# mfkiwl/GPS-JAMMING

Hardware: AMD Instinct MI355X
Metric: Msamples/s uint8 I/Q through PSD+TDOA xcorr (higher is better)
Workload: dtype f32

## Files before the change

gps-jamming_amd/csrc/k_scan.hip:

```cpp
#include <type_traits>

#include "gj_common.h"

namespace gj {

constexpr int kScanThreads = 256;
constexpr size_t kScanTile = 65536;

__device__ __forceinline__ void acc_moments(const uint4& q, unsigned& s2, unsigned& s1) {
    s2 = __builtin_amdgcn_udot4(q.x, q.x, s2, false);
    s2 = __builtin_amdgcn_udot4(q.y, q.y, s2, false);
    s2 = __builtin_amdgcn_udot4(q.z, q.z, s2, false);
    s2 = __builtin_amdgcn_udot4(q.w, q.w, s2, false);
    s1 = __builtin_amdgcn_udot4(q.x, 0x01010101u, s1, false);
    s1 = __builtin_amdgcn_udot4(q.y, 0x01010101u, s1, false);
    s1 = __builtin_amdgcn_udot4(q.z, 0x01010101u, s1, false);
    s1 = __builtin_amdgcn_udot4(q.w, 0x01010101u, s1, false);
}

__device__ __forceinline__ void block_byte_moments(const uint8_t* __restrict__ p, size_t begin, size_t end,
                                                   unsigned long long& s2_out, unsigned long long& s1_out) {
    __shared__ unsigned long long red[2][kScanThreads / 64];
    const int tid = threadIdx.x;
    unsigned s2 = 0, s1 = 0;
    size_t a0 = (begin + 15) & ~size_t(15);
    size_t a1 = end & ~size_t(15);
    if (a0 > a1) { a0 = end; a1 = end; }
    if (begin + tid < a0) { unsigned u = p[begin + tid]; s2 += u * u; s1 += u; }
    if (a1 + tid < end && a1 >= a0) { unsigned u = p[a1 + tid]; s2 += u * u; s1 += u; }
    const uint4* v = reinterpret_cast<const uint4*>(p + a0);
    const size_t nvec = (a1 - a0) >> 4;
    size_t i = tid;
    for (; i + 3 * kScanThreads < nvec; i += 4 * kScanThreads) {
        uint4 w0 = v[i], w1 = v[i + kScanThreads], w2 = v[i + 2 * kScanThreads], w3 = v[i + 3 * kScanThreads];
        acc_moments(w0, s2, s1); acc_moments(w1, s2, s1); acc_moments(w2, s2, s1); acc_moments(w3, s2, s1);
    }
    for (; i < nvec; i += kScanThreads) {
        uint4 w0 = v[i];
        acc_moments(w0, s2, s1);
    }
    unsigned long long t2 = wave_sum_u64(s2), t1 = wave_sum_u64(s1);
    if ((tid & 63) == 0) { red[0][tid >> 6] = t2; red[1][tid >> 6] = t1; }
    __syncthreads();
    if (tid == 0) {
        s2_out = red[0][0] + red[0][1] + red[0][2] + red[0][3];
        s1_out = red[1][0] + red[1][1] + red[1][2] + red[1][3];
    }
    __syncthreads();
}

__device__ __forceinline__ float power_from_moments(unsigned long long s2, unsigned long long s1, size_t npairs,
                                                    float eps, int o2) {
    const long long S = 4ll * (long long)s2 - 4ll * o2 * (long long)s1 + (long long)o2 * o2 * (long long)(2 * npairs);
    const float mean = (float)((double)S / (4.0 * (double)npairs));
    return mean + eps;
}

__device__ __forceinline__ float power_from_msum(unsigned long long S, size_t npairs, float eps) {
    const float mean = (float)((double)S / (4.0 * (double)npairs));
    return mean + eps;
}

__global__ __launch_bounds__(kScanThreads) void chunk_power_kernel(const uint8_t* __restrict__ iq, size_t nbytes,
                                                                   size_t chunk_bytes, unsigned tiles_per_chunk,
                                                                   float eps, int flags, float* __restrict__ power,
                                                                   unsigned long long* __restrict__ acc, int o2) {
    const size_t c = blockIdx.x / tiles_per_chunk;
    const unsigned t = blockIdx.x % tiles_per_chunk;
    const size_t off = c * chunk_bytes;
    const size_t len = (nbytes - off < chunk_bytes) ? nbytes - off : chunk_bytes;
    const size_t npairs = len >> 1;
    if ((flags & GJ_CP_ODD_CHUNK_ZERO) && ((len & 1) || len == 0)) {
        if (t == 0 && threadIdx.x == 0) power[c] = 0.0f;
        return;
    }
    if (npairs == 0) {
        if (t == 0 && threadIdx.x == 0) power[c] = __builtin_nanf("");
        return;
    }
    const size_t use_end = off + 2 * npairs;
    size_t b = off + (size_t)t * kScanTile;
    size_t e = b + kScanTile;
    if (e > use_end) e = use_end;
    if (b > e) b = e;
    unsigned long long s2 = 0, s1 = 0;
    block_byte_moments(iq, b, e, s2, s1);
    if (threadIdx.x == 0) {
        if (tiles_per_chunk == 1) {
            power[c] = power_from_moments(s2, s1, npairs, eps, o2);
        } else {
            atomicAdd(&acc[2 * c], s2);
            atomicAdd(&acc[2 * c + 1], s1);
        }
    }
}

__global__ void chunk_power_finalize_kernel(const unsigned long long* __restrict__ acc, size_t nchunks, size_t nbytes,
                                            size_t chunk_bytes, float eps, int flags, float* __restrict__ power,
                                            int o2, bool msum = false) {
    const size_t c = blockIdx.x * (size_t)blockDim.x + threadIdx.x;
    if (c >= nchunks) return;
    const size_t off = c * chunk_bytes;
    const size_t len = (nbytes - off < chunk_bytes) ? nbytes - off : chunk_bytes;
    const size_t npairs = len >> 1;
    if ((flags & GJ_CP_ODD_CHUNK_ZERO) && ((len & 1) || len == 0)) return;
    if (npairs == 0) return;
    power[c] = msum ? power_from_msum(acc[2 * c], npairs, eps) : power_from_moments(acc[2 * c], acc[2 * c + 1], npairs, eps, o2);
}

int launch_chunk_power(gj_ctx* ctx, const uint8_t* d_iq, size_t nbytes, size_t chunk_bytes, float eps, int flags,
                       float* d_power) {
    if (chunk_bytes == 0) return fail(ctx, GJ_ERR_INVALID, "chunk_bytes must be > 0");
    const size_t nchunks = gj_chunk_count(nbytes, chunk_bytes);
    if (nchunks == 0) return GJ_OK;
    const size_t tiles = (chunk_bytes + kScanTile - 1) / kScanTile;
    if (nchunks * tiles > 0x7fffffffull) return fail(ctx, GJ_ERR_UNSUPPORTED, "too many tiles");
    unsigned long long* acc = nullptr;
    if (tiles > 1) {
        int rc = ensure_workspace(ctx, nchunks * 16);
        if (rc) return rc;
        acc = reinterpret_cast<unsigned long long*>(ctx->ws);
        GJ_HIP(ctx, hipMemsetAsync(acc, 0, nchunks * 16, ctx->stream));
    }
    hipLaunchKernelGGL(chunk_power_kernel, dim3((unsigned)(nchunks * tiles)), dim3(kScanThreads), 0, ctx->stream, d_iq,
                       nbytes, chunk_bytes, (unsigned)tiles, eps, flags, d_power, acc, ctx->off2);
    GJ_LAUNCH_CHECK(ctx);
    if (tiles > 1) {
        hipLaunchKernelGGL(chunk_power_finalize_kernel, dim3((unsigned)((nchunks + 255) / 256)), dim3(256), 0,
                           ctx->stream, acc, nchunks, nbytes, chunk_bytes, eps, flags, d_power, ctx->off2);
        GJ_LAUNCH_CHECK(ctx);
    }
    return GJ_OK;
}

__device__ __forceinline__ unsigned float_key(float f) {
    unsigned b = __float_as_uint(f);
    return (b & 0x80000000u) ? ~b : (b | 0x80000000u);
}
__device__ __forceinline__ float key_float(unsigned k) {
    return __uint_as_float((k & 0x80000000u) ? (k & 0x7fffffffu) : ~k);
}

constexpr int kThrThreads = 256;
constexpr int kThrPerThread = 64;
constexpr int kThrCache = kThrThreads * kThrPerThread;

struct ThrShared {
    unsigned hist[256];
    unsigned wave_tot[4];
    unsigned digit, rest;
    unsigned nan_flag;
    unsigned count_le;
    unsigned next_key;
    unsigned long long above;
// ... 183 lines not shown

constexpr size_t kAmpTileSamples = kScanTile / 2;

struct AmpTile {
    double sum;
    long long first;
};

__device__ double block_sum_f64(double v, double* sh ) {
    v = wave_sum_f64(v);
    __syncthreads();
    if ((threadIdx.x & 63) == 0) sh[threadIdx.x >> 6] = v;
    __syncthreads();
    double t = 0.0;
    for (unsigned k = 0; k < blockDim.x / 64; ++k) t += sh[k];
    return t;
}

__device__ long long amp_block_first(const AmpTile* __restrict__ tiles, size_t ntiles, long long* first_s) {
    if (threadIdx.x == 0) *first_s = 0x7fffffffffffffffll;
    __syncthreads();
    long long f = 0x7fffffffffffffffll;
    for (size_t t = threadIdx.x; t < ntiles; t += 16 * (size_t)blockDim.x) {
        long long v[16];
#pragma unroll
        for (int k = 0; k < 16; ++k) {
            const size_t tt = t + (size_t)k * blockDim.x;
            v[k] = tt < ntiles ? tiles[tt].first : 0x7fffffffffffffffll;
        }
#pragma unroll
        for (int k = 0; k < 16; ++k) f = v[k] < f ? v[k] : f;
    }
    if (f != 0x7fffffffffffffffll) atomicMin(first_s, f);
    __syncthreads();
    return *first_s;
}

__device__ double amp_block_tail(const uint8_t* __restrict__ iq, size_t nsamples, const AmpTile* __restrict__ tiles,
                                 long long first, Unpack up, double* sh) {
    const size_t t0 = (size_t)first / kAmpTileSamples;
    if ((size_t)first == t0 * kAmpTileSamples) return tiles[t0].sum;
    const size_t e0 = ((t0 + 1) * kAmpTileSamples < nsamples) ? (t0 + 1) * kAmpTileSamples : nsamples;
    double acc = 0.0;
    for (size_t s = (size_t)first + threadIdx.x; s < e0; s += blockDim.x) acc += (double)amp_of(iq[2 * s], iq[2 * s + 1], up);
    return block_sum_f64(acc, sh);
}

__device__ double amp_block_total(const AmpTile* __restrict__ tiles, size_t ntiles, size_t t0, double* sh) {
    double acc = 0.0;
    for (size_t t = t0 + 1 + threadIdx.x; t < ntiles; t += 16 * (size_t)blockDim.x) {
        double v[16];
#pragma unroll
        for (int k = 0; k < 16; ++k) {
            const size_t tt = t + (size_t)k * blockDim.x;
            v[k] = tt < ntiles ? tiles[tt].sum : 0.0;
        }
#pragma unroll
        for (int g = 0; g < 2; ++g) {
            if (t + (size_t)(8 * g) * blockDim.x < ntiles)
                acc += ((v[8 * g] + v[8 * g + 1]) + (v[8 * g + 2] + v[8 * g + 3])) + ((v[8 * g + 4] + v[8 * g + 5]) + (v[8 * g + 6] + v[8 * g + 7]));
        }
    }
    return block_sum_f64(acc, sh);
}

static inline bool power_edge_value(size_t nchunks, size_t nbytes, size_t chunk_bytes, int flags, float* val) {
    if (!nchunks) return false;
    const size_t len = nbytes - (nchunks - 1) * chunk_bytes;
    if ((flags & GJ_CP_ODD_CHUNK_ZERO) && (len & 1)) { *val = 0.0f; return true; }
    if ((len >> 1) == 0) { *val = __builtin_nanf(""); return true; }
    return false;
}
__device__ __forceinline__ void amp_combine_body(const AmpTile* __restrict__ tiles, size_t ntiles,
                                                 const gj_amp_part* __restrict__ parts, int n_parts, size_t nsamples,
                                                 gj_amp_stats* __restrict__ out, double* sh) {
    long long first = 0x7fffffffffffffffll;
    double tail = 0.0;
    for (int p = 0; p < n_parts; ++p)
        if (parts[p].first_index >= 0 && parts[p].first_index < first) { first = parts[p].first_index; tail = parts[p].tail; }
    if (first == 0x7fffffffffffffffll) {
        if (threadIdx.x == 0) {
            out->first_index = -1; out->count = 0; out->sum = 0.0; out->mean = 0.f; out->reserved = 0.f;
        }
        return;
    }
    const double behind = amp_block_total(tiles, ntiles, (size_t)first / kAmpTileSamples, sh);
    if (threadIdx.x == 0) {
        const double total = behind + tail;
        const unsigned long long cnt = nsamples - (size_t)first;
        out->first_index = first;
        out->count = cnt;
        out->sum = total;
        out->mean = (float)(total / (double)cnt);
        out->reserved = 0.f;
    }
}

__global__ __launch_bounds__(256) void amp_combine_kernel(const AmpTile* __restrict__ tiles, size_t ntiles,
                                                           const gj_amp_part* __restrict__ parts, int n_parts,
                                                           size_t nsamples, gj_amp_stats* __restrict__ out) {
    __shared__ double sh[16];
    amp_combine_body(tiles, ntiles, parts, n_parts, nsamples, out, sh);
}

__global__ __launch_bounds__(kThrThreads) __attribute__((amdgpu_num_vgpr(104))) void combine_stats_kernel(
    const gj_combine_capture* __restrict__ caps, int n_captures, float pct, float ratio) {
    __shared__ ThrShared sh_thr;
    __shared__ double sh_amp[16];
    const int b = blockIdx.x;
    if (b < n_captures) {
        const gj_combine_capture c = caps[b];
        power_threshold_body(c.d_power, (size_t)c.n_chunks, pct, ratio, c.d_stats, nullptr, sh_thr);
    } else {
        const gj_combine_capture c = caps[b - n_captures];
        amp_combine_body(static_cast<const AmpTile*>(c.d_tiles), (size_t)c.n_tiles, c.d_amp_parts, c.n_parts,
                         (size_t)(c.total_bytes / 2), c.d_amp, sh_amp);
        if (threadIdx.x == 0) onset_combine(c.d_onset_parts, c.n_parts, c.d_onset);
    }
}

int launch_combine_stats(gj_ctx* ctx, const gj_combine_capture* d_caps, int n_captures, float pct, float rise_db) {
    const float ratio = (float)pow(10.0, (double)rise_db / 10.0);
    hipLaunchKernelGGL(combine_stats_kernel, dim3(2u * (unsigned)n_captures), dim3(kThrThreads), 0, ctx->stream, d_caps,
                       n_captures, pct, ratio);
    GJ_LAUNCH_CHECK(ctx);
    return GJ_OK;
}

constexpr int kOnsetOut = 2048;
constexpr int kOnsetMaxWin = 8192;

struct OnsetScratch {
    unsigned long long noise_S;
    float noise;
    float thr;
};

constexpr double kOnsetGuard = 1e-6;

__device__ __forceinline__ int onset_pad(int k) { return k + (k >> 5); }

typedef short gj_short2 __attribute__((ext_vector_type(2)));

__device__ __forceinline__ int wave_sum_lane63(int v) {
    v += __builtin_amdgcn_update_dpp(0, v, 0xB1, 0xf, 0xf, false);
    v += __builtin_amdgcn_update_dpp(0, v, 0x4E, 0xf, 0xf, false);
    v += __builtin_amdgcn_update_dpp(0, v, 0x141, 0xf, 0xf, false);
    v += __builtin_amdgcn_update_dpp(0, v, 0x140, 0xf, 0xf, false);
    v += __builtin_amdgcn_update_dpp(0, v, 0x142, 0xa, 0xf, false);
    v += __builtin_amdgcn_update_dpp(0, v, 0x143, 0xc, 0xf, false);
    return v;
}


template <bool TRACK_FIRST>
__global__ __launch_bounds__(kScanThreads) void stream_scan_kernel(const uint8_t* __restrict__ iq, size_t nsamples,
                                                                   size_t nbytes, size_t chunk_bytes,
                                                                   unsigned tiles_per_chunk, float eps, int flags,
                                                                   float* __restrict__ power,
                                                                   unsigned long long* __restrict__ acc, float thr,
                                                                   AmpTile* __restrict__ tiles,
                                                                   unsigned* __restrict__ cblk, Unpack up,
                                                                   unsigned skip_tiles, unsigned tile_base,
                                                                   unsigned noise_block, const uint8_t* __restrict__ noise_src,
                                                                   int noise_samples, OnsetScratch* __restrict__ sc) {
    if (blockIdx.x == noise_block) {
        unsigned long long s2 = 0, s1 = 0;
        block_byte_moments(noise_src, 0, (size_t)2 * noise_samples, s2, s1);
        if (threadIdx.x == 0)
            sc->noise_S = (unsigned long long)(4ll * (long long)s2 - 4ll * up.off2 * (long long)s1 + (long long)up.off2 * up.off2 * (2ll * noise_samples));
        return;
    }
    __shared__ unsigned long long red_m[2][kScanThreads / 64];
    __shared__ double red_s[kScanThreads / 64];
    __shared__ long long red_f[kScanThreads / 64];
    const int tid = threadIdx.x;
    const size_t t = (size_t)blockIdx.x + tile_base;
    const size_t b0 = t * kScanTile;
    const size_t use_end = 2 * nsamples;
    const size_t b1 = (b0 + kScanTile < use_end) ? b0 + kScanTile : use_end;
    const size_t nvec = (b1 - b0) >> 4;
    const uint4* v = reinterpret_cast<const uint4*>(iq + b0);
    unsigned S = 0;
    double sum = 0.0;
    long long first = 0x7fffffffffffffffll;
    unsigned k2 = 0x00020002u, km255 = pk_minus_off2(up.off2);
    asm volatile("" : "+v"(k2), "+v"(km255));
    auto body = [&](const uint4& q, unsigned i, const bool live) {
        const unsigned ws[4] = {q.x, q.y, q.z, q.w};
        int m[8];
#pragma unroll
        for (int k = 0; k < 4; ++k) {
            m[2 * k] = msq_of_half<0>(ws[k], k2, km255);
            m[2 * k + 1] = msq_of_half<1>(ws[k], k2, km255);
        }
        float part = 0.f;
#pragma unroll
        for (int k = 0; k < 8; ++k) {
            const float r = __fsqrt_rn((float)m[k]);
            part += r;
            if constexpr (TRACK_FIRST) {
                const long long idx = (long long)((b0 >> 1) + (size_t)i * 8 + k);
                if (live && r * up.half_scale > thr && idx < first) first = idx;
            }
        }
        const unsigned m8 = live ? (unsigned)(((m[0] + m[1]) + (m[2] + m[3])) + ((m[4] + m[5]) + (m[6] + m[7]))) : 0u;
        S += m8;
        const int c512 = wave_sum_lane63((int)m8);
        if ((tid & 63) == 63) cblk[(b0 >> 10) + (i >> 6)] = (unsigned)c512;
        sum += (double)(live ? part : 0.f);
    };
    if (nvec == kScanTile / 16) {
        for (unsigned i = tid; i < (unsigned)(kScanTile / 16); i += 4 * kScanThreads) {
            const uint4 q0 = v[i], q1 = v[i + kScanThreads], q2 = v[i + 2 * kScanThreads], q3 = v[i + 3 * kScanThreads];
            body(q0, i, true);
            body(q1, i + kScanThreads, true);
            body(q2, i + 2 * kScanThreads, true);
            body(q3, i + 3 * kScanThreads, true);
        }
    } else {
        const unsigned lane = tid & 63;
        for (unsigned ib = (unsigned)tid - lane; ib < (unsigned)nvec; ib += kScanThreads) {
            const unsigned i = ib + lane;
            const bool live = i < (unsigned)nvec;
            const uint4 q = live ? v[i] : uint4{0u, 0u, 0u, 0u};
            body(q, i, live);
        }
    }
    if (tid == 0 && (b0 + (nvec << 4)) < b1) {
        unsigned c = 0;
        for (size_t n = (b0 >> 1) + nvec * 8; 2 * n < b1; ++n) {
            const unsigned ui = iq[2 * n], uq = iq[2 * n + 1];
            const unsigned mm = m_of(ui, uq, up.off2);
            S += mm;
            c += mm;
            const float r = __fsqrt_rn((float)mm);
            sum += (double)r;
            if (TRACK_FIRST && r * up.half_scale > thr && (long long)n < first) first = (long long)n;
        }
        (void)c;
    }
    if (b1 == use_end && (b1 & 1023) != 0) {
        __syncthreads();
        if (tid < 64) {
            const size_t jb = (b1 - 1) >> 10;
            int c = 0;
            for (size_t n = jb * 512 + tid; n < nsamples; n += 64) c += (int)m_of(iq[2 * n], iq[2 * n + 1], up.off2);
            c = group_sum_dpp<64>(c);
            if (tid == 0) cblk[jb] = (unsigned)c;
        }
    }
    if constexpr (!TRACK_FIRST) {
        if (tid == 0 && b1 > b0) first = (long long)(b0 >> 1);
    }
    const unsigned long long mS = wave_sum_u64(S);
    sum = wave_sum_f64(sum);
#pragma unroll
    for (int off = 32; off > 0; off >>= 1) {
        const long long o = __shfl_xor(first, off, 64);
        first = o < first ? o : first;
    }
    if ((tid & 63) == 0) { red_m[0][tid >> 6] = mS; red_s[tid >> 6] = sum; red_f[tid >> 6] = first; }
    __syncthreads();
    if (tid == 0 && t >= skip_tiles) {
        const unsigned long long tS = red_m[0][0] + red_m[0][1] + red_m[0][2] + red_m[0][3];
        AmpTile at;
        at.sum = ((red_s[0] + red_s[1]) + (red_s[2] + red_s[3])) * (double)up.half_scale;
        long long f = red_f[0];
        for (int k = 1; k < 4; ++k) f = red_f[k] < f ? red_f[k] : f;
        at.first = (f == 0x7fffffffffffffffll) ? f : f - (long long)((size_t)skip_tiles * (kScanTile / 2));
        const size_t to = t - skip_tiles;
        tiles[to] = at;
        const size_t c = to / tiles_per_chunk;
        const size_t off = c * chunk_bytes;
        const size_t len = (nbytes - off < chunk_bytes) ? nbytes - off : chunk_bytes;
        const bool zero_rule = (flags & GJ_CP_ODD_CHUNK_ZERO) && ((len & 1) || len == 0);
        if (tiles_per_chunk == 1) {
            power[c] = zero_rule ? 0.0f : ((len >> 1) ? power_from_msum(tS, len >> 1, eps) : __builtin_nanf(""));
        } else {
            atomicAdd(&acc[2 * c], tS);
        }
    }
}

constexpr size_t kTailSlotBytes = 256u << 10;
constexpr size_t kTailPrioBytes = 256u << 20;
constexpr int kTailBlocks = 2048;
constexpr int kTailHalo = (kOnsetMaxWin + 510) / 512 + 1;
constexpr int kTailPre = kTailBlocks + kTailHalo + (kTailBlocks + kTailHalo) / 32 + 8;

struct TailRec {
    unsigned long long first;
    unsigned long long guard;
    unsigned below;
    unsigned pad;
};

struct TailArgs {
    const uint8_t* iq;
    unsigned long long nsamples;
    long long sample0;
    unsigned long long total_samples;
    unsigned long long slot_nsamples;
    int has_thr, is_part, valid, has_slot, hi_prio;
    float* power;
    unsigned long long nchunks;
    float pct, ratio;
    float* stats;
    uint8_t* mask;
    const uint8_t* own_iq;
    unsigned long long own_samples, own_tiles;
    const AmpTile* tiles;
    gj_amp_stats* amp;
    gj_amp_part* amp_part;
    long long own_sample0;
    int window, noise_samples, noise_in_scratch;
    float factor;
    const unsigned* cblk;
    OnsetScratch* sc;
    TailRec* rec;
    unsigned* arrive;
    unsigned nct;
    gj_onset* onset;
    uint8_t* slot;
    unsigned long long slice_samples;
    Unpack up;
};

struct TailShared {
    unsigned long long r64[2][kScanThreads / 64];
    unsigned r32[kScanThreads / 64];
    unsigned long long b64[2];
    unsigned b32;
    int last;
    long long start;
};

__device__ __forceinline__ unsigned long long block_min_u64(unsigned long long v, TailShared& sh, int slot) {
#pragma unroll
    for (int off = 32; off > 0; off >>= 1) {
        const unsigned long long o = __shfl_xor(v, off, 64);
        v = o < v ? o : v;
    }
    if ((threadIdx.x & 63) == 0) sh.r64[slot][threadIdx.x >> 6] = v;
    __syncthreads();
    unsigned long long r = sh.r64[slot][0];
#pragma unroll
    for (int k = 1; k < kScanThreads / 64; ++k) r = sh.r64[slot][k] < r ? sh.r64[slot][k] : r;
    __syncthreads();
    return r;
}
__device__ __forceinline__ unsigned block_max_u32(unsigned v, TailShared& sh) {
#pragma unroll
    for (int off = 32; off > 0; off >>= 1) {
        const unsigned o = __shfl_xor(v, off, 64);
        v = o > v ? o : v;
    }
    if ((threadIdx.x & 63) == 0) sh.r32[threadIdx.x >> 6] = v;
    __syncthreads();
    unsigned r = sh.r32[0];
#pragma unroll
    for (int k = 1; k < kScanThreads / 64; ++k) r = sh.r32[k] > r ? sh.r32[k] : r;
    __syncthreads();
    return r;
}
__device__ __forceinline__ unsigned long long block_sum_u64(unsigned long long v, TailShared& sh) {
    v = wave_sum_u64(v);
    if ((threadIdx.x & 63) == 0) sh.r64[0][threadIdx.x >> 6] = v;
    __syncthreads();
    unsigned long long r = 0;
#pragma unroll
    for (int k = 0; k < kScanThreads / 64; ++k) r += sh.r64[0][k];
    __syncthreads();
    return r;
}

__device__ __forceinline__ void block_min2_max(unsigned long long& a, unsigned long long& b, unsigned& c, TailShared& sh) {
#pragma unroll
    for (int off = 32; off > 0; off >>= 1) {
        const unsigned long long oa = __shfl_xor(a, off, 64), ob = __shfl_xor(b, off, 64);
        const unsigned oc = __shfl_xor(c, off, 64);
        a = oa < a ? oa : a;
        b = ob < b ? ob : b;
        c = oc > c ? oc : c;
    }
    if ((threadIdx.x & 63) == 0) { sh.r64[0][threadIdx.x >> 6] = a; sh.r64[1][threadIdx.x >> 6] = b; sh.r32[threadIdx.x >> 6] = c; }
    __syncthreads();
    a = sh.r64[0][0]; b = sh.r64[1][0]; c = sh.r32[0];
#pragma unroll
    for (int k = 1; k < kScanThreads / 64; ++k) {
        a = sh.r64[0][k] < a ? sh.r64[0][k] : a;
        b = sh.r64[1][k] < b ? sh.r64[1][k] : b;
        c = sh.r32[k] > c ? sh.r32[k] : c;
// ... 118 lines not shown
            }
        }
        unsigned long long hit = best, hit_lo = best_lo;
        unsigned b = 0;
#pragma unroll
        for (int i = 0; i < kOnsetOut / kScanThreads; ++i) {
            const int k = tid + i * kScanThreads;
            if (k < npos && o0 + k < best) b = Sv[i] > b ? Sv[i] : b;
        }
        block_min2_max(hit, hit_lo, b, sh);
        if (hit != ~0ull) {
            b = 0;
#pragma unroll
            for (int i = 0; i < kOnsetOut / kScanThreads; ++i) {
                const int k = tid + i * kScanThreads;
                if (k < npos && o0 + k < hit) b = Sv[i] > b ? Sv[i] : b;
            }
            b = block_max_u32(b, sh);
        }
        below = b > below ? b : below;
        if (hit_lo != ~0ull && guard == ~0ull) guard = hit_lo;
        if (hit != ~0ull) { first = hit; break; }
        kstart = k1 + (npos + 511) / 512;
    }
    if (tid == 0) {
        TailRec r;
        r.first = first; r.guard = guard; r.below = below; r.pad = 0;
        A.rec[w] = r;
    }
}

__device__ void tail_onset_finish(const TailArgs& A, TailShared& sh) {
    const int tid = threadIdx.x;
    const int window = A.window;
    if (A.valid) {
        unsigned long long wmin = ~0ull;
        for (unsigned w = tid; w < A.nct; w += kScanThreads)
            if (A.rec[w].first != ~0ull) { wmin = w; break; }
        const unsigned long long wstar = block_min_u64(wmin, sh, 0);
        const bool found = wstar != ~0ull;
        const unsigned wlast = found ? (unsigned)wstar : A.nct - 1;
        unsigned below = 0;
        unsigned long long guard = ~0ull;
        for (unsigned w = tid; w <= wlast; w += kScanThreads) {
            const TailRec r = A.rec[w];
            below = r.below > below ? r.below : below;
            guard = r.guard < guard ? r.guard : guard;
        }
        below = block_max_u32(below, sh);
        guard = block_min_u64(guard, sh, 1);
        const unsigned long long i0 = found ? A.rec[wstar].first : 0ull;
        unsigned long long S = 0;
        if (found)
            for (int k = tid; k < window; k += kScanThreads) S += m_of(A.iq[2 * (i0 + k)], A.iq[2 * (i0 + k) + 1], A.up.off2);
        S = block_sum_u64(S, sh);
        if (tid == 0) {
            const double thr = (double)A.sc->thr, scale = 0.25 / (double)window;
            gj_onset o;
            o.start_index = found ? A.sample0 + (long long)i0 + window / 2 : -1;
            o.noise_power = A.sc->noise;
            o.threshold = A.sc->thr;
            o.margin_hit = found ? (float)(((double)S * scale - thr) / thr) : 0.f;
            o.margin_before = (float)((thr - (double)below * scale) / thr);
            unsigned long long ig = guard;
            if (found && i0 < ig) ig = i0;
            o.guard_index = ig != ~0ull ? A.sample0 + (long long)ig + window / 2 : -1;
            *A.onset = o;
            sh.start = o.start_index;
        }
    } else if (tid == 0) {
        gj_onset o;
        o.start_index = -1; o.noise_power = 0.f; o.threshold = 0.f; o.margin_hit = 0.f; o.margin_before = 0.f; o.guard_index = -1;
        *A.onset = o;
        sh.start = -1;
    }
    __syncthreads();
    if (A.has_slot)
        tdoa_slot_body(A.iq, (size_t)A.slot_nsamples, sh.start, (size_t)A.slice_samples, A.slot, A.sample0, (size_t)A.total_samples,
                       (size_t)tid, (size_t)kScanThreads, tid == 0);
}

__global__ __launch_bounds__(kScanThreads) void scan_tail_kernel(TailArgs A) {
    __shared__ ThrShared sh_thr;
    __shared__ double sh_amp[16];
    __shared__ long long first_s;
    __shared__ TailShared sh;
    __shared__ unsigned pre_c[kTailPre];
    __shared__ unsigned thread_tot[kScanThreads];
    extern __shared__ unsigned pre_x[];
    const int tid = threadIdx.x;
    unsigned b = blockIdx.x;
    if (A.hi_prio) __builtin_amdgcn_s_setprio(3);
    if (A.has_thr) {
        if (b == 0) {
            power_threshold_body(A.power, (size_t)A.nchunks, A.pct, A.ratio, A.stats, A.mask, sh_thr);
            return;
        }
        --b;
    }
    if (b == 0) {
        const long long first = amp_block_first(A.tiles, (size_t)A.own_tiles, &first_s);
        if (first == 0x7fffffffffffffffll) {
            if (tid == 0) {
                if (A.is_part) { A.amp_part->first_index = -1; A.amp_part->count = 0; A.amp_part->sum = 0.0; A.amp_part->tail = 0.0; }
                else { A.amp->first_index = -1; A.amp->count = 0; A.amp->sum = 0.0; A.amp->mean = 0.f; A.amp->reserved = 0.f; }
            }
            return;
        }
        const double tail = amp_block_tail(A.own_iq, (size_t)A.own_samples, A.tiles, first, A.up, sh_amp);
        const double behind = amp_block_total(A.tiles, (size_t)A.own_tiles, (size_t)first / kAmpTileSamples, sh_amp);
        if (tid == 0) {
            const unsigned long long cnt = A.own_samples - (size_t)first;
            if (A.is_part) {
                A.amp_part->first_index = A.own_sample0 + first;
                A.amp_part->count = cnt;
                A.amp_part->sum = behind + tail;
                A.amp_part->tail = tail;
            } else {
                const double total = behind + tail;
                A.amp->first_index = first;
                A.amp->count = cnt;
                A.amp->sum = total;
                A.amp->mean = (float)(total / (double)cnt);
                A.amp->reserved = 0.f;
            }
        }
        return;
    }
    --b;
    if (A.valid) tail_onset_range(A, b, pre_c, thread_tot, pre_x, sh);
    if (tid == 0) {
        const unsigned ticket = arrive_release(A.arrive);
        const int last = ticket == A.nct - 1;
        if (last) last_arriver_acquire(A.arrive);
        sh.last = last;
    }
    __syncthreads();
    if (!sh.last) return;
    tail_onset_finish(A, sh);
}

struct ScanPart {
    size_t halo_bytes;
    long long buf_sample0;
    const uint8_t* d_noise;
    size_t total_samples;
    AmpTile* d_tiles;
    gj_amp_part* d_amp;
};

struct ScanState {
    const uint8_t* d_iq;
    size_t nbytes, chunk_bytes, own_bytes, nsamples, own_samples, ntiles, skip, own_tiles, nchunks, tpc, noise_bytes;
    float eps, rssi_threshold, factor;
    int flags, noise_samples, window, valid;
    bool noise_here, track, is_part;
    float* d_power;
    gj_amp_stats* d_amp;
    gj_onset* d_onset;
    ScanPart part;
    size_t off_tiles, off_acc, off_blk, off_rec;
    unsigned nct;
};
static_assert(sizeof(ScanState) <= sizeof(ScanJob::state), "ScanJob::state too small");

bool scan_fusable(const uint8_t* d_iq, size_t nbytes, size_t chunk_bytes) {
    return chunk_bytes >= kScanTile && chunk_bytes % kScanTile == 0 && (reinterpret_cast<uintptr_t>(d_iq) & 15) == 0 && nbytes >= 2;
}

static int scan_begin_impl(gj_ctx* ctx, const uint8_t* d_iq, size_t nbytes, size_t chunk_bytes, float eps, int flags,
                           float* d_power, float rssi_threshold, gj_amp_stats* d_amp, int noise_samples, int window,
                           float factor, gj_onset* d_onset, const ScanPart* part, ScanJob& job) {
    if (noise_samples <= 0 || window <= 0) return fail(ctx, GJ_ERR_INVALID, "noise_samples and window must be > 0");
    if (window > kOnsetMaxWin) return fail(ctx, GJ_ERR_UNSUPPORTED, "window > %d", kOnsetMaxWin);
    ScanState st;
    memset(&st, 0, sizeof(st));
    st.d_iq = d_iq; st.nbytes = nbytes; st.chunk_bytes = chunk_bytes; st.eps = eps; st.flags = flags; st.d_power = d_power;
    st.rssi_threshold = rssi_threshold; st.d_amp = d_amp; st.noise_samples = noise_samples; st.window = window;
    st.factor = factor; st.d_onset = d_onset;
    st.is_part = part != nullptr;
    if (part) st.part = *part;
    const size_t halo = part ? part->halo_bytes : 0;
    st.own_bytes = nbytes - halo;
    st.nsamples = nbytes / 2;
    st.own_samples = st.own_bytes / 2;
    st.ntiles = (2 * st.nsamples + kScanTile - 1) / kScanTile;
    st.skip = halo / kScanTile;
    st.own_tiles = st.ntiles - st.skip;
    st.nchunks = gj_chunk_count(st.own_bytes, chunk_bytes);
    st.tpc = chunk_bytes / kScanTile;
    const size_t nblk = (st.nsamples + 511) / 512;
    if (st.ntiles > 0x7fffffffull) return fail(ctx, GJ_ERR_UNSUPPORTED, "capture too long");
    st.off_tiles = 256;
    st.off_acc = st.off_tiles + (part ? 0 : align_up((st.own_tiles + 1) * sizeof(AmpTile), 256));
    st.off_blk = st.off_acc + align_up(st.nchunks * 16, 256);
    const size_t total_samples = part ? part->total_samples : st.nsamples;
    st.valid = d_onset && total_samples >= (size_t)noise_samples + (size_t)window && st.nsamples >= (size_t)window;
    st.noise_bytes = (size_t)2 * noise_samples;
    st.noise_here = !part || (part->buf_sample0 == 0 && st.noise_bytes <= nbytes);
    if (st.valid && !st.noise_here && !part->d_noise)
        return fail(ctx, GJ_ERR_INVALID, "this part does not hold the capture's noise span (%zu bytes): d_noise is required", st.noise_bytes);
    const Unpack upk = unpack_of(ctx);
    const bool all_hit = (ctx->off2 & 1) && (sqrtf(2.0f) * upk.half_scale > rssi_threshold);
    st.track = !all_hit;
    job.ntiles = st.ntiles;
    job.nchunks = st.nchunks;
    st.off_rec = align_up(st.off_blk + (nblk + 16) * sizeof(unsigned), 256);
    {
        const size_t nout = st.valid ? st.nsamples - (size_t)window + 1 : 0;
        const size_t nct = st.valid ? ((nout + 511) / 512 + kTailBlocks - 1) / kTailBlocks : (d_onset ? 1 : 0);
        if (nct > 0x7ffffff0ull) return fail(ctx, GJ_ERR_UNSUPPORTED, "capture too long");
        st.nct = (unsigned)nct;
    }
    memcpy(job.state, &st, sizeof(st));
    job.ws_bytes = align_up(st.off_rec + (size_t)st.nct * sizeof(TailRec), 256);
    job.ws = nullptr;
    return GJ_OK;
}

int scan_begin(gj_ctx* ctx, const uint8_t* d_iq, size_t nbytes, size_t chunk_bytes, float eps, int flags, float* d_power,
               float rssi_threshold, gj_amp_stats* d_amp, int noise_samples, int window, float factor, gj_onset* d_onset,
               ScanJob& job) {
    if (!scan_fusable(d_iq, nbytes, chunk_bytes)) return fail(ctx, GJ_ERR_UNSUPPORTED, "the fused scan needs chunk_bytes to be a multiple of 65536 and a 16-byte aligned capture");
    return scan_begin_impl(ctx, d_iq, nbytes, chunk_bytes, eps, flags, d_power, rssi_threshold, d_amp, noise_samples, window,
                           factor, d_onset, nullptr, job);
}

int scan_start(gj_ctx* ctx, ScanJob& job) {
    ScanState st;
    memcpy(&st, job.state, sizeof(st));
    if (st.tpc > 1) GJ_HIP(ctx, hipMemsetAsync(job.ws + st.off_acc, 0, st.nchunks * 16, ctx->stream));
    return GJ_OK;
}

int scan_range(gj_ctx* ctx, const ScanJob& job, size_t tile0, size_t tile1) {
    ScanState st;
    memcpy(&st, job.state, sizeof(st));
    if (tile1 > st.ntiles) tile1 = st.ntiles;
    if (tile0 >= tile1) return GJ_OK;
    OnsetScratch* sc = reinterpret_cast<OnsetScratch*>(job.ws);
    AmpTile* tiles = st.is_part ? st.part.d_tiles : reinterpret_cast<AmpTile*>(job.ws + st.off_tiles);
    unsigned long long* acc = reinterpret_cast<unsigned long long*>(job.ws + st.off_acc);
    unsigned* cblk = reinterpret_cast<unsigned*>(job.ws + st.off_blk);
    const Unpack upk = unpack_of(ctx);
    const unsigned n = (unsigned)(tile1 - tile0);
    const bool noise_wg = st.valid && !st.noise_here && tile0 == 0;
    const unsigned noise_block = noise_wg ? n : 0xffffffffu;
    const dim3 grid(n + (noise_wg ? 1u : 0u));
    if (st.track)
        hipLaunchKernelGGL(stream_scan_kernel<true>, grid, dim3(kScanThreads), 0, ctx->stream, st.d_iq, st.nsamples,
                           st.own_bytes, st.chunk_bytes, (unsigned)st.tpc, st.eps, st.flags, st.d_power, acc, st.rssi_threshold,
                           tiles, cblk, upk, (unsigned)st.skip, (unsigned)tile0, noise_block, st.part.d_noise, st.noise_samples, sc);
    else
        hipLaunchKernelGGL(stream_scan_kernel<false>, grid, dim3(kScanThreads), 0, ctx->stream, st.d_iq, st.nsamples,
                           st.own_bytes, st.chunk_bytes, (unsigned)st.tpc, st.eps, st.flags, st.d_power, acc, st.rssi_threshold,
                           tiles, cblk, upk, (unsigned)st.skip, (unsigned)tile0, noise_block, st.part.d_noise, st.noise_samples, sc);
    GJ_LAUNCH_CHECK(ctx);
    return GJ_OK;
}

int scan_end(gj_ctx* ctx, const ScanJob& job, const ScanExtra* extra) {
    ScanState st;
    memcpy(&st, job.state, sizeof(st));
    OnsetScratch* sc = reinterpret_cast<OnsetScratch*>(job.ws);
    AmpTile* tiles = st.is_part ? st.part.d_tiles : reinterpret_cast<AmpTile*>(job.ws + st.off_tiles);
    unsigned long long* acc = reinterpret_cast<unsigned long long*>(job.ws + st.off_acc);
    const size_t halo = st.is_part ? st.part.halo_bytes : 0;
    if (st.tpc > 1) {
        hipLaunchKernelGGL(chunk_power_finalize_kernel, dim3((unsigned)((st.nchunks + 255) / 256)), dim3(256), 0,
                           ctx->stream, acc, st.nchunks, st.own_bytes, st.chunk_bytes, st.eps, st.flags, st.d_power, ctx->off2, true);
        GJ_LAUNCH_CHECK(ctx);
    }
    {
        float edge;
        if (st.d_power && power_edge_value(st.nchunks, st.own_bytes, st.chunk_bytes, st.flags, &edge)) {
            unsigned bits;
            memcpy(&bits, &edge, 4);
            GJ_HIP(ctx, hipMemsetD32Async(reinterpret_cast<hipDeviceptr_t>(st.d_power + (st.nchunks - 1)), (int)bits, 1, ctx->stream));
        }
    }
    TailArgs A;
    memset(&A, 0, sizeof(A));
    A.iq = st.d_iq;
    A.nsamples = st.nsamples;
    A.sample0 = st.is_part ? st.part.buf_sample0 : 0ll;
    A.total_samples = st.is_part ? st.part.total_samples : st.nsamples;
    A.is_part = st.is_part;
    A.valid = st.valid;
    A.power = st.d_power;
    A.nchunks = st.nchunks;
    if (extra && extra->d_stats && st.nchunks) {
        A.has_thr = 1;
        A.pct = extra->pct;
        A.ratio = (float)pow(10.0, (double)extra->rise_db / 10.0);
        A.stats = extra->d_stats;
        A.mask = extra->d_mask;
    }
    A.own_iq = st.d_iq + halo;
    A.own_samples = st.own_samples;
    A.own_tiles = st.own_tiles;
    A.tiles = tiles;
    A.amp = st.d_amp;
    A.amp_part = st.part.d_amp;
    A.own_sample0 = A.sample0 + (long long)(halo / 2);
    A.window = st.window;
    A.noise_samples = st.noise_samples;
    A.noise_in_scratch = st.valid && !st.noise_here;
    A.factor = st.factor;
    A.cblk = reinterpret_cast<const unsigned*>(job.ws + st.off_blk);
    A.sc = sc;
    A.rec = reinterpret_cast<TailRec*>(job.ws + st.off_rec);
    A.arrive = ctx->d_sync + kSyncTail;
    A.nct = st.nct;
    A.onset = st.d_onset;
    if (extra && extra->d_slot) {
        if (extra->slice_samples < 1) return fail(ctx, GJ_ERR_INVALID, "n_samples must be >= 1");
        if ((reinterpret_cast<uintptr_t>(extra->d_slot) & 15) != 0) return fail(ctx, GJ_ERR_INVALID, "slot must be 16-byte aligned");
        A.slot = extra->d_slot;
        A.slice_samples = extra->slice_samples;
        A.slot_nsamples = extra->slot_buf_bytes ? extra->slot_buf_bytes / 2 : st.nsamples;
        A.has_slot = 2 * extra->slice_samples <= kTailSlotBytes;
    }
    A.hi_prio = st.nbytes <= kTailPrioBytes;
    A.up = unpack_of(ctx);
    const int needx = kOnsetOut + st.window - 1;
    const size_t dyn = (size_t)(needx + needx / 32 + 8) * sizeof(unsigned);
    const unsigned grid = (A.has_thr ? 1u : 0u) + 1u + st.nct;
    hipLaunchKernelGGL(scan_tail_kernel, dim3(grid), dim3(kScanThreads), dyn, ctx->stream, A);
    GJ_LAUNCH_CHECK(ctx);
    if (A.slot && !A.has_slot)
        return launch_tdoa_slot(ctx, st.d_iq, 2 * (size_t)A.slot_nsamples, &st.d_onset->start_index, (size_t)A.slice_samples, A.slot,
                                A.sample0, (size_t)A.total_samples);
    return GJ_OK;
}

static int stream_scan_impl(gj_ctx* ctx, const uint8_t* d_iq, size_t nbytes, size_t chunk_bytes, float eps, int flags,
                            float* d_power, float rssi_threshold, gj_amp_stats* d_amp, int noise_samples, int window,
                            float factor, gj_onset* d_onset, const ScanPart* part, const ScanExtra* extra = nullptr) {
    ScanJob job;
    int rc = scan_begin_impl(ctx, d_iq, nbytes, chunk_bytes, eps, flags, d_power, rssi_threshold, d_amp, noise_samples, window,
                             factor, d_onset, part, job);
    if (rc) return rc;
    rc = ensure_workspace(ctx, job.ws_bytes);
    if (rc) return rc;
    job.ws = ctx->ws;
    rc = scan_start(ctx, job);
    if (!rc) rc = scan_range(ctx, job, 0, job.ntiles);
    if (!rc) rc = scan_end(ctx, job, extra);
    return rc;
}

int launch_amp_onset(gj_ctx* ctx, const uint8_t* d_iq, size_t nbytes, float rssi_threshold, gj_amp_stats* d_amp,
                     int noise_samples, int window, float factor, gj_onset* d_onset) {
    if (!d_amp && !d_onset) return GJ_OK;
    if (!d_onset) { noise_samples = 1; window = 1; factor = 1.f; }
    if (!d_amp) rssi_threshold = -1.0f;
    const bool aligned = (reinterpret_cast<uintptr_t>(d_iq) & 15) == 0;
    ScanJob job;
    int rc = scan_begin_impl(ctx, d_iq, nbytes, kScanTile, 0.f, 0, nullptr, rssi_threshold, d_amp, noise_samples, window, factor,
                             d_onset, nullptr, job);
    if (rc) return rc;
    const size_t off_power = job.ws_bytes;
    const size_t off_amp = off_power + align_up((job.nchunks + 1) * sizeof(float), 256);
    const size_t off_copy = off_amp + 256;
    rc = ensure_workspace(ctx, off_copy + (aligned ? 0 : align_up(nbytes, 256)));
    if (rc) return rc;
    if (!aligned && nbytes) {
        GJ_HIP(ctx, hipMemcpyAsync(ctx->ws + off_copy, d_iq, nbytes, hipMemcpyDeviceToDevice, ctx->stream));
        d_iq = ctx->ws + off_copy;
    }
    rc = scan_begin_impl(ctx, d_iq, nbytes, kScanTile, 0.f, 0, reinterpret_cast<float*>(ctx->ws + off_power), rssi_threshold,
                         d_amp ? d_amp : reinterpret_cast<gj_amp_stats*>(ctx->ws + off_amp), noise_samples, window, factor, d_onset,
                         nullptr, job);
    if (rc) return rc;
    job.ws = ctx->ws;
    rc = scan_start(ctx, job);
    if (!rc) rc = scan_range(ctx, job, 0, job.ntiles);
    if (!rc) rc = scan_end(ctx, job, nullptr);
    return rc;
}

int launch_amp_stats(gj_ctx* ctx, const uint8_t* d_iq, size_t nbytes, float threshold, gj_amp_stats* d_out) {
    return launch_amp_onset(ctx, d_iq, nbytes, threshold, d_out, 0, 0, 0.f, nullptr);
}

int launch_onset(gj_ctx* ctx, const uint8_t* d_iq, size_t nbytes, int noise_samples, int window, float factor,
                 gj_onset* d_out) {
    return launch_amp_onset(ctx, d_iq, nbytes, 0.f, nullptr, noise_samples, window, factor, d_out);
}

int launch_stream_scan(gj_ctx* ctx, const uint8_t* d_iq, size_t nbytes, size_t chunk_bytes, float eps, int flags,
                       float* d_power, float rssi_threshold, gj_amp_stats* d_amp, int noise_samples, int window,
                       float factor, gj_onset* d_onset, const ScanExtra* extra) {
    if (!scan_fusable(d_iq, nbytes, chunk_bytes)) {
        int rc = launch_chunk_power(ctx, d_iq, nbytes, chunk_bytes, eps, flags, d_power);
        if (!rc) rc = launch_amp_onset(ctx, d_iq, nbytes, rssi_threshold, d_amp, noise_samples, window, factor, d_onset);
        if (!rc && extra && extra->d_stats && gj_chunk_count(nbytes, chunk_bytes))
            rc = launch_power_threshold(ctx, d_power, gj_chunk_count(nbytes, chunk_bytes), extra->pct, extra->rise_db, extra->d_stats, extra->d_mask);
        if (!rc && extra && extra->d_slot)
            rc = launch_tdoa_slot(ctx, d_iq, nbytes, &d_onset->start_index, extra->slice_samples, extra->d_slot);
        return rc;
    }
    return stream_scan_impl(ctx, d_iq, nbytes, chunk_bytes, eps, flags, d_power, rssi_threshold, d_amp, noise_samples,
                            window, factor, d_onset, nullptr, extra);
}

int launch_part_scan(gj_ctx* ctx, const gj_part_view& v, size_t chunk_bytes, float eps, int flags, float* d_power,
                     float rssi_threshold, void* d_tiles, gj_amp_part* d_amp, int noise_samples, int window, float factor,
// ... 73 lines not shown
```

Measured before the change: 408,300.

## Precompute integer magnitude-squared threshold and batch DPP wave sums in scan kernel

Replaces the per-sample float sqrt, multiply and compare used for first-hit tracking with an integer compare against a threshold on m, found on the host by binary search. That search reproduces the float rounding, including the subnormal half_scale case. Each lane now records only its first hit and then disables further checks, instead of doing a 64-bit index min per sample. The four per-iteration DPP wave reductions are interleaved so their latencies overlap. The risk is exact-equivalence bugs in the threshold derivation, and the restructured loop may use more registers.

```diff
diff --git a/gps-jamming_amd/csrc/amp_hit.h b/gps-jamming_amd/csrc/amp_hit.h
--- /dev/null
+++ b/gps-jamming_amd/csrc/amp_hit.h
@@ -0,0 +1,52 @@
+#pragma once
+
+#include <climits>
+#include <cmath>
+#include <cstdint>
+#include <cstring>
+
+namespace gj {
+
+inline double amp_hit_widen(float f) {
+    uint32_t b;
+    memcpy(&b, &f, sizeof(b));
+    const int e = (int)((b >> 23) & 0xffu);
+    const uint32_t man = b & 0x7fffffu;
+    double v;
+    if (e == 0xff) v = man ? (double)NAN : (double)INFINITY;
+    else v = e ? ldexp((double)(man | 0x800000u), e - 150) : ldexp((double)man, -149);
+    return (b >> 31) ? -v : v;
+}
+
+inline bool amp_hit_is_subnormal(float f) {
+    uint32_t b;
+    memcpy(&b, &f, sizeof(b));
+    return ((b >> 23) & 0xffu) == 0 && (b & 0x7fffffu) != 0;
+}
+
+inline bool amp_hit_pred(int m, float half_scale, float thr) {
+    volatile float r = sqrtf((float)m);
+    if (amp_hit_is_subnormal(half_scale)) {
+        const double q = ldexp((double)r * amp_hit_widen(half_scale), 149);
+        double n = floor(q);
+        const double frac = q - n;
+        if (frac > 0.5 || (frac == 0.5 && fmod(n, 2.0) != 0.0)) n += 1.0;
+        return ldexp(n, -149) > amp_hit_widen(thr);
+    }
+    volatile float a = r * half_scale;
+    return a > thr;
+}
+
+inline int amp_hit_m(int off2, float half_scale, float thr) {
+    const int c = off2 > 510 - off2 ? off2 : 510 - off2;
+    int lo = 0, hi = 2 * c * c;
+    if (!amp_hit_pred(hi, half_scale, thr)) return INT_MAX;
+    while (lo < hi) {
+        const int mid = lo + (hi - lo) / 2;
+        if (amp_hit_pred(mid, half_scale, thr)) hi = mid;
+        else lo = mid + 1;
+    }
+    return lo;
+}
+
+}
diff --git a/gps-jamming_amd/csrc/k_scan.hip b/gps-jamming_amd/csrc/k_scan.hip
--- a/gps-jamming_amd/csrc/k_scan.hip
+++ b/gps-jamming_amd/csrc/k_scan.hip
@@ -1,5 +1,6 @@
 #include <type_traits>
 
+#include "amp_hit.h"
 #include "gj_common.h"
 
 namespace gj {
@@ -489,13 +490,29 @@
     return v;
 }
 
+template <int CTRL, int ROWS>
+__device__ __forceinline__ void dpp_add_x4(int (&v)[4]) {
+    int t[4];
+#pragma unroll
+    for (int j = 0; j < 4; ++j) t[j] = __builtin_amdgcn_update_dpp(0, v[j], CTRL, ROWS, 0xf, false);
+#pragma unroll
+    for (int j = 0; j < 4; ++j) v[j] += t[j];
+}
+__device__ __forceinline__ void wave_sum_lane63_x4(int (&v)[4]) {
+    dpp_add_x4<0xB1, 0xf>(v);
+    dpp_add_x4<0x4E, 0xf>(v);
+    dpp_add_x4<0x141, 0xf>(v);
+    dpp_add_x4<0x140, 0xf>(v);
+    dpp_add_x4<0x142, 0xa>(v);
+    dpp_add_x4<0x143, 0xc>(v);
+}
 
 template <bool TRACK_FIRST>
 __global__ __launch_bounds__(kScanThreads) void stream_scan_kernel(const uint8_t* __restrict__ iq, size_t nsamples,
                                                                    size_t nbytes, size_t chunk_bytes,
                                                                    unsigned tiles_per_chunk, float eps, int flags,
                                                                    float* __restrict__ power,
-                                                                   unsigned long long* __restrict__ acc, float thr,
+                                                                   unsigned long long* __restrict__ acc, int m_thr,
                                                                    AmpTile* __restrict__ tiles,
                                                                    unsigned* __restrict__ cblk, Unpack up,
                                                                    unsigned skip_tiles, unsigned tile_base,
@@ -520,40 +537,55 @@
     const uint4* v = reinterpret_cast<const uint4*>(iq + b0);
     unsigned S = 0;
     double sum = 0.0;
-    long long first = 0x7fffffffffffffffll;
+    unsigned first_local = ~0u;
+    int mthr_lane = m_thr;
     unsigned k2 = 0x00020002u, km255 = pk_minus_off2(up.off2);
     asm volatile("" : "+v"(k2), "+v"(km255));
-    auto body = [&](const uint4& q, unsigned i, const bool live) {
+    auto msq8 = [&](const uint4& q, int (&m)[8]) {
         const unsigned ws[4] = {q.x, q.y, q.z, q.w};
-        int m[8];
 #pragma unroll
         for (int k = 0; k < 4; ++k) {
             m[2 * k] = msq_of_half<0>(ws[k], k2, km255);
             m[2 * k + 1] = msq_of_half<1>(ws[k], k2, km255);
         }
+    };
+    auto track = [&](const int (&m)[8], unsigned i, const bool live) {
+        const int mx = max(max(max(max(max(max(max(m[0], m[1]), m[2]), m[3]), m[4]), m[5]), m[6]), m[7]);
+        if (live && mx >= mthr_lane) {
+            unsigned k = 7;
+#pragma unroll
+            for (int j = 6; j >= 0; --j) k = (m[j] >= mthr_lane) ? (unsigned)j : k;
+            first_local = i * 8 + k;
+            mthr_lane = 0x7fffffff;
+        }
+    };
+    auto amp8 = [&](const int (&m)[8]) {
         float part = 0.f;
 #pragma unroll
-        for (int k = 0; k < 8; ++k) {
-            const float r = __fsqrt_rn((float)m[k]);
-            part += r;
-            if constexpr (TRACK_FIRST) {
-                const long long idx = (long long)((b0 >> 1) + (size_t)i * 8 + k);
-                if (live && r * up.half_scale > thr && idx < first) first = idx;
-            }
-        }
-        const unsigned m8 = live ? (unsigned)(((m[0] + m[1]) + (m[2] + m[3])) + ((m[4] + m[5]) + (m[6] + m[7]))) : 0u;
-        S += m8;
-        const int c512 = wave_sum_lane63((int)m8);
-        if ((tid & 63) == 63) cblk[(b0 >> 10) + (i >> 6)] = (unsigned)c512;
-        sum += (double)(live ? part : 0.f);
+        for (int k = 0; k < 8; ++k) part += __fsqrt_rn((float)m[k]);
+        return part;
     };
+    auto msum8 = [&](const int (&m)[8]) { return (unsigned)(((m[0] + m[1]) + (m[2] + m[3])) + ((m[4] + m[5]) + (m[6] + m[7]))); };
     if (nvec == kScanTile / 16) {
         for (unsigned i = tid; i < (unsigned)(kScanTile / 16); i += 4 * kScanThreads) {
-            const uint4 q0 = v[i], q1 = v[i + kScanThreads], q2 = v[i + 2 * kScanThreads], q3 = v[i + 3 * kScanThreads];
-            body(q0, i, true);
-            body(q1, i + kScanThreads, true);
-            body(q2, i + 2 * kScanThreads, true);
-            body(q3, i + 3 * kScanThreads, true);
+            const uint4 q[4] = {v[i], v[i + kScanThreads], v[i + 2 * kScanThreads], v[i + 3 * kScanThreads]};
+            int c512[4];
+#pragma unroll
+            for (int j = 0; j < 4; ++j) {
+                int m[8];
+                msq8(q[j], m);
+                if constexpr (TRACK_FIRST) track(m, i + j * kScanThreads, true);
+                const unsigned m8 = msum8(m);
+                S += m8;
+                c512[j] = (int)m8;
+                sum += (double)amp8(m);
+            }
+            wave_sum_lane63_x4(c512);
+            if ((tid & 63) == 63) {
+                unsigned* cb = cblk + (b0 >> 10) + (i >> 6);
+#pragma unroll
+                for (int j = 0; j < 4; ++j) cb[j * (kScanThreads / 64)] = (unsigned)c512[j];
+            }
         }
     } else {
         const unsigned lane = tid & 63;
@@ -561,21 +593,26 @@
             const unsigned i = ib + lane;
             const bool live = i < (unsigned)nvec;
             const uint4 q = live ? v[i] : uint4{0u, 0u, 0u, 0u};
-            body(q, i, live);
-        }
-    }
+            int m[8];
+            msq8(q, m);
+            if constexpr (TRACK_FIRST) track(m, i, live);
+            const unsigned m8 = live ? msum8(m) : 0u;
+            S += m8;
+            const int c512 = wave_sum_lane63((int)m8);
+            if (lane == 63) cblk[(b0 >> 10) + (i >> 6)] = (unsigned)c512;
+            const float part = amp8(m);
+            sum += (double)(live ? part : 0.f);
+        }
+    }
+    long long first = (first_local != ~0u) ? (long long)((b0 >> 1) + first_local) : 0x7fffffffffffffffll;
     if (tid == 0 && (b0 + (nvec << 4)) < b1) {
-        unsigned c = 0;
         for (size_t n = (b0 >> 1) + nvec * 8; 2 * n < b1; ++n) {
             const unsigned ui = iq[2 * n], uq = iq[2 * n + 1];
             const unsigned mm = m_of(ui, uq, up.off2);
             S += mm;
-            c += mm;
-            const float r = __fsqrt_rn((float)mm);
-            sum += (double)r;
-            if (TRACK_FIRST && r * up.half_scale > thr && (long long)n < first) first = (long long)n;
-        }
-        (void)c;
+            sum += (double)__fsqrt_rn((float)mm);
+            if (TRACK_FIRST && (int)mm >= m_thr && (long long)n < first) first = (long long)n;
+        }
     }
     if (b1 == use_end && (b1 & 1023) != 0) {
         __syncthreads();
@@ -1000,8 +1037,9 @@
 struct ScanState {
     const uint8_t* d_iq;
     size_t nbytes, chunk_bytes, own_bytes, nsamples, own_samples, ntiles, skip, own_tiles, nchunks, tpc, noise_bytes;
-    float eps, rssi_threshold, factor;
+    float eps, factor;
     int flags, noise_samples, window, valid;
+    int m_thr;
     bool noise_here, track, is_part;
     float* d_power;
     gj_amp_stats* d_amp;
@@ -1024,7 +1062,7 @@
     ScanState st;
     memset(&st, 0, sizeof(st));
     st.d_iq = d_iq; st.nbytes = nbytes; st.chunk_bytes = chunk_bytes; st.eps = eps; st.flags = flags; st.d_power = d_power;
-    st.rssi_threshold = rssi_threshold; st.d_amp = d_amp; st.noise_samples = noise_samples; st.window = window;
+    st.d_amp = d_amp; st.noise_samples = noise_samples; st.window = window;
     st.factor = factor; st.d_onset = d_onset;
     st.is_part = part != nullptr;
     if (part) st.part = *part;
@@ -1049,7 +1087,8 @@
     if (st.valid && !st.noise_here && !part->d_noise)
         return fail(ctx, GJ_ERR_INVALID, "this part does not hold the capture's noise span (%zu bytes): d_noise is required", st.noise_bytes);
     const Unpack upk = unpack_of(ctx);
-    const bool all_hit = (ctx->off2 & 1) && (sqrtf(2.0f) * upk.half_scale > rssi_threshold);
+    st.m_thr = amp_hit_m(upk.off2, upk.half_scale, rssi_threshold);
+    const bool all_hit = (ctx->off2 & 1) && st.m_thr <= 2;
     st.track = !all_hit;
     job.ntiles = st.ntiles;
     job.nchunks = st.nchunks;
@@ -1097,11 +1136,11 @@
     const dim3 grid(n + (noise_wg ? 1u : 0u));
     if (st.track)
         hipLaunchKernelGGL(stream_scan_kernel<true>, grid, dim3(kScanThreads), 0, ctx->stream, st.d_iq, st.nsamples,
-                           st.own_bytes, st.chunk_bytes, (unsigned)st.tpc, st.eps, st.flags, st.d_power, acc, st.rssi_threshold,
+                           st.own_bytes, st.chunk_bytes, (unsigned)st.tpc, st.eps, st.flags, st.d_power, acc, st.m_thr,
                            tiles, cblk, upk, (unsigned)st.skip, (unsigned)tile0, noise_block, st.part.d_noise, st.noise_samples, sc);
     else
         hipLaunchKernelGGL(stream_scan_kernel<false>, grid, dim3(kScanThreads), 0, ctx->stream, st.d_iq, st.nsamples,
-                           st.own_bytes, st.chunk_bytes, (unsigned)st.tpc, st.eps, st.flags, st.d_power, acc, st.rssi_threshold,
+                           st.own_bytes, st.chunk_bytes, (unsigned)st.tpc, st.eps, st.flags, st.d_power, acc, st.m_thr,
                            tiles, cblk, upk, (unsigned)st.skip, (unsigned)tile0, noise_block, st.part.d_noise, st.noise_samples, sc);
     GJ_LAUNCH_CHECK(ctx);
     return GJ_OK;
```

After: 405,400. No clear change (-0.7%).
